# daisy9542/yolo-puncture

Measured on AMD Instinct MI355X. Metric: images/sec, higher is better.
Workload: dtype bf16

## Files before the change

yolo-puncture_amd/csrc/common.h:

```cpp
#pragma once
#include <hip/hip_runtime.h>
#include <stdint.h>
#include <string>
#include <vector>

namespace yp {

enum DType { DT_BF16 = 0, DT_F32 = 1 };
enum Act { ACT_NONE = 0, ACT_SILU = 1, ACT_RELU = 2 };

enum OpKind {
    OP_STEM = 0,
    OP_CONV = 1,
    OP_DWCONV = 2,
    OP_POOL5 = 3,
    OP_UPSAMPLE = 4,
    OP_ATTN = 5,
    OP_HEAD = 6,
    OP_CONVT = 7,
    OP_AMAX = 9,
    OP_POOL3 = 8,
};

struct View {
// ... 40 lines not shown
    int nlev = 0;
    double flops = 0, bytes = 0;
    std::string kernel;
    int cfg = -1;
    int fuse_dw = -1;
    bool fused = false;
    bool skip = false;
    int fuse_pre = -1;
    bool fused2 = false;
    int stem_op = -1;
    bool fused3 = false;
    int fold_up = -1;
    bool folded = false;
    int c2f_m1 = -1, c2f_m2 = -1;
    bool fused4 = false;
    int scd_pre = -1;
    bool fused5 = false;
    int fuse_tail = -1, tail_amax = -1;
    bool fused6 = false;
    int amax_post = -1;
    bool fused8 = false;
    int pw_pre = -1;
    bool fused7 = false;
    bool pw_store = false;
    int lane = 0;
    bool nms = false;
    int hb_box[3][3] = {{-1, -1, -1}, {-1, -1, -1}, {-1, -1, -1}}, hb_cf[3][3] = {{-1, -1, -1}, {-1, -1, -1}, {-1, -1, -1}};
    bool sparse_box = false, sparse_cf = false;
};

// ... 50 lines not shown
bool frontend_valid(const FrontParams& p);
hipError_t launch_frontend(const FrontParams& p, hipStream_t st);

struct C2fParams {
    const void* x; int x_stride, x_coff; size_t x_bytes;
    int B, H, W, C;
    const void* w1; const float* bias1; int act1, Kpad1; size_t w1_bytes;
    const void* w2; const float* bias2; int act2, Kpad2; size_t w2_bytes;
    int shortcut;
    const void* w3; const float* bias3; int act3, Kpad3, Cout; size_t w3_bytes;
    void* y; int y_stride, y_coff; size_t y_bytes;
    unsigned long long* clk;
};
bool c2f_fused_valid(const C2fParams& p);

struct ScdParams {
    const void* x; int x_stride, x_coff; size_t x_bytes; int B, H, W, K;
    const void* w1; const float* bias1; int act1, Kpad1, C; size_t w1_bytes;
    const void* wd; const float* biasd; int actd;
    void* y; int y_stride, y_coff; size_t y_bytes; int Ho, Wo;
    unsigned long long* clk;
};
bool scdown_fused_valid(const ScdParams& p);
const char* scdown_fused_kernel_name(const ScdParams& p);
bool scdown_stream_valid(const ScdParams& p);
const char* scdown_stream_kernel_name(const ScdParams& p);
hipError_t launch_scdown_stream(const ScdParams& p, hipStream_t st);
hipError_t launch_scdown_fused(const ScdParams& p, hipStream_t st);
hipError_t launch_c2f_fused(const C2fParams& p, hipStream_t st);

struct PoolParams {
    const void* x; int x_stride, x_coff;
    void* y; int y_stride, y_coff;
    int B, H, W, C;
};

struct UpParams {
    const void* x; int x_stride, x_coff;
    void* y; int y_stride, y_coff;
    int B, H, W, C;
};

struct AttnParams {
    const void* qkv; int q_stride, q_coff;
// ... 225 lines not shown
```

yolo-puncture_amd/csrc/engine.hip:

```cpp
#include "../../include/yolop.h"
#include "common.h"
#include <algorithm>
#include <array>
#include <chrono>

#include <cmath>
#include <cstdarg>
#include <cstdio>
#include <cstring>
#include <cstdlib>
#include <dlfcn.h>
#include <fcntl.h>
#include <fstream>
#include <map>
#include <sstream>
#include <memory>

using namespace yp;

static thread_local char g_err[512] = "";
static int fail(int code, const char* fmt, ...) {
    va_list ap;
    va_start(ap, fmt);
    vsnprintf(g_err, sizeof(g_err), fmt, ap);
// ... 17 lines not shown
    std::map<std::string, int> wmap;
    bool finalized = false;
    int pB = 0, pH = 0, pW = 0;
    bool planned = false, allocated = false;
    void* arena = nullptr;
    size_t arena_bytes = 0;
    int proto_t = -1;
    void* mask_ws = nullptr;
    void* head_ws = nullptr;
    size_t head_ws_bytes = 0;
    size_t mask_ws_bytes = 0;
    bool use_graph = false;
    bool graph_auto = false;
    std::map<std::array<int, 3>, bool> auto_replay;
    bool fuse = true;
    bool tail = false;
    bool sparse_head = true;
    void* sp_ws = nullptr; size_t sp_ws_bytes = 0;
    bool tune = true;
    int tune_source = 0;
    hipStream_t own_stream = nullptr;
    hipEvent_t ev_in = nullptr;
    hipGraphExec_t gexec = nullptr;
    hipGraph_t gsrc = nullptr;
    bool use_lanes = true;
    int n_captures = 0;
    int g_nodes = 0, g_edges = 0, g_edges_expected = 0;
    hipStream_t last_stream = nullptr; bool have_last = false;
    struct LaneStep { int op = -1; std::vector<int> waits; bool fork = false; bool record = false; };
    std::vector<LaneStep> lane_steps;
// ... 81 lines not shown
    int sdiv_of(View v) const { return e.tensors[v.t].sdiv; }

    void c2f(const std::string& p, View in, View out, int c2, int n, bool shortcut, bool cib, bool lk) {
        const int c = c2 / 2, sd = sdiv_of(in);
        const int Y = tensor(p + ".cat", (2 + n) * c, sd);
        int m1 = -1;
        conv(p + ".cv1", in, View{Y, 0, 2 * c}, 1, 1, ACT_SILU);
        for (int j = 0; j < n; ++j) {
            const View x{Y, (1 + j) * c, c}, y{Y, (2 + j) * c, c};
            const std::string q = p + ".m." + std::to_string(j);
            const View res = shortcut ? x : View{};
            if (!cib) {
                const int t = tensor(q + ".cv1", c, sd);
                conv(q + ".cv1", x, full(t), 3, 1, ACT_SILU);
                conv(q + ".cv2", full(t), y, 3, 1, ACT_SILU, res);
                if (n == 1) m1 = (int)e.ops.size() - 2;
            } else {
                const int t0 = tensor(q + ".cv1.0", c, sd), t1 = tensor(q + ".cv1.1", 2 * c, sd);
                const int t2 = tensor(q + ".cv1.2", 2 * c, sd), t3 = tensor(q + ".cv1.3", c, sd);
                dwconv(q + ".cv1.0", x, full(t0), 3, 1, ACT_SILU);
                conv(q + ".cv1.1", full(t0), full(t1), 1, 1, ACT_SILU);
                dwconv(q + ".cv1.2", full(t1), full(t2), lk ? 7 : 3, 1, ACT_SILU);
                conv(q + ".cv1.3", full(t2), full(t3), 1, 1, ACT_SILU);
                dwconv(q + ".cv1.4", full(t3), y, 3, 1, ACT_SILU, res);
            }
        }
        conv(p + ".cv2", full(Y), out, 1, 1, ACT_SILU);
        if (m1 >= 0) { e.ops.back().c2f_m1 = m1; e.ops.back().c2f_m2 = m1 + 1; }
    }
    void bottleneck(const std::string& q, View x, View y, int ch, bool shortcut) {
        const int t = tensor(q + ".cv1", ch, sdiv_of(x));
        conv(q + ".cv1", x, full(t), 3, 1, ACT_SILU);
        conv(q + ".cv2", full(t), y, 3, 1, ACT_SILU, shortcut ? x : View{});
    }
    void c3k2(const std::string& p, View in, View out, int c2, int n, bool c3k, double e) {
        const int c = (int)(c2 * e), sd = sdiv_of(in);
        const int Y = tensor(p + ".cat", (2 + n) * c, sd);
        conv(p + ".cv1", in, View{Y, 0, 2 * c}, 1, 1, ACT_SILU);
        for (int j = 0; j < n; ++j) {
            const View x{Y, (1 + j) * c, c}, y{Y, (2 + j) * c, c};
            const std::string q = p + ".m." + std::to_string(j);
            const int c_ = c / 2;
            if (!c3k) { bottleneck(q, x, y, c_, true); continue; }
            const int Z = tensor(q + ".cat", 2 * c_, sd);
            const int a0 = tensor(q + ".cv1", c_, sd), a1 = tensor(q + ".m.0", c_, sd);
            conv(q + ".cv1", x, full(a0), 1, 1, ACT_SILU);
            bottleneck(q + ".m.0", full(a0), full(a1), c_, true);
            bottleneck(q + ".m.1", full(a1), View{Z, 0, c_}, c_, true);
// ... 439 lines not shown
        if (d.in.coff < pw.out.coff || d.in.coff + d.in.C > pw.out.coff + pw.out.C) continue;
        if (e.tensors[pw.out.t].f32 || e.tensors[d.out.t].f32) continue;
        d.pw_pre = c;
    }
    return YP_OK;
}

static ConvParams conv_params(const yp_engine& e, const Op& o);
static void drop_graph(yp_engine& e) {
    if (e.gexec) { (void)hipGraphExecDestroy(e.gexec); e.gexec = nullptr; }
    if (e.gsrc) { (void)hipGraphDestroy(e.gsrc); e.gsrc = nullptr; }
}
static DwPwParams dwpw_params(const yp_engine& e, const Op& c);
static FrontParams front_params(const yp_engine& e, const Op& o, const uint8_t* img);
static C2fParams c2f_params(const yp_engine& e, const Op& o);
static ScdParams scd_params(const yp_engine& e, const Op& o);
static PwSpParams pwsp_params(const yp_engine& e, const Op& o);
static ClsOutParams cls_out_params(const yp_engine& e, const Op& o);
static bool views_overlap(const View& a, const View& b);
static size_t tensor_elem_bytes(const yp_engine& e, const TensorDesc& t) { return (t.f32 || e.dtype == DT_F32) ? 4 : 2; }

struct SparseWs {
    size_t sel, wlist, wcount, thr, box, cf, pcount, plist, t0box, t0cf, total;
    int plist_off[3], plist_cap[3];
    size_t t0_off[3];
    size_t rows;
};
static SparseWs sparse_ws_layout(int B, int max_det, const int (&HWl)[3]) {
    SparseWs w{};
    size_t off = 0;
// ... 75 lines not shown
            o.bytes += (double)w.cout * w.cin_g * w.k * w.k * es;
            if (o.kind == OP_STEM) o.bytes += (double)B * H * W * 3;
        } else if (o.kind == OP_ATTN) {
            const TensorDesc& ti = e.tensors[o.in.t];
            const double Nn = (double)ti.H * ti.W;
            o.flops = 2.0 * B * o.nh * Nn * Nn * (o.kd + o.hd);
        } else if (o.kind == OP_HEAD) {
            o.bytes = 0;
            for (int l = 0; l < 3; ++l) o.bytes += (o.amax[l].t >= 0) ? vbytes(o.amax[l]) : vbytes(o.cls[l]);
            o.bytes += (double)B * e.desc.max_det * (e.desc.nc + 64 + 6 + 1) * 4;
        }
    }
    e.pB = B; e.pH = H; e.pW = W; e.planned = true; e.allocated = false; e.warmed = false;
    for (auto& o : e.ops) o.cfg = -1;
    static const char* kn[] = {"stem_kernel", "", "dwconv_kernel", "pool5_kernel", "upsample2_kernel", "attention_kernel", "head_select_kernel", "", "sppf_pool3_kernel", "anchor_max_level_kernel"};
    for (auto& o : e.ops) { o.fused = false; o.skip = false; o.folded = false; o.fused2 = false; o.fused3 = false; o.fused4 = false; o.fused5 = false; o.fused6 = false; o.fused7 = false; o.fused8 = false; o.pw_store = false; o.sparse_box = false; o.sparse_cf = false; }
    static const bool no_fold = [] { const char* v = std::getenv("YOLOP_NO_FOLD"); return v && *v == '1'; }();
    for (auto& o : e.ops) {
        if (o.kind != OP_CONV || o.fold_up < 0 || e.dtype != DT_BF16 || no_fold) continue;
        o.folded = true;
        const ConvParams q = conv_params(e, o);
        bool any = false;
        for (int c = 0; c < conv_dma_p_num_cfgs() && !any; ++c) any = conv_dma_p_cfg_valid(q, c);
        if (any) e.ops[o.fold_up].skip = true;
        else o.folded = false;
    }
    for (auto& o : e.ops) {
        if (o.kind == OP_CONV && o.fuse_pre >= 0 && e.dtype == DT_BF16 && e.fuse) {
            o.fused2 = true;
            const int c = conv_halo_s2_pw_cfg(conv_params(e, o));
            if (c >= 0) {
// ... 54 lines not shown
            q.x_bytes = (size_t)B * q.H * q.W * q.x_stride * 2;
            if (dwconv_mfma_valid(q, e.dtype)) snprintf(buf, sizeof(buf), "dwconv_mfma_kernel<%d,%s>", o.k, B * (q.C / 32) >= 256 ? "false" : "true");
            else if (o.k == 3 && o.s == 1) snprintf(buf, sizeof(buf), "dwconv_row_kernel<%s,3,1,4>", t);
            else if (o.k == 3 && o.s == 2) snprintf(buf, sizeof(buf), "dwconv_row_kernel<%s,3,2,2>", t);
            else if (o.k == 7 && o.s == 1) snprintf(buf, sizeof(buf), "dwconv_row_kernel<%s,7,1,2>", t);
            else snprintf(buf, sizeof(buf), "dwconv_kernel<%s>", t);
            o.kernel = buf;
        } else if (o.kind == OP_STEM) {
            char buf[64];
            if (e.dtype == DT_BF16) snprintf(buf, sizeof(buf), "stem_mfma_kernel<%d>", o.out.C / 16);
            else snprintf(buf, sizeof(buf), "stem_kernel<f32>");
            o.kernel = buf;
        } else if (o.kind == OP_POOL3 && e.dtype == DT_BF16 && (o.in.C & 31) == 0) o.kernel = "sppf_pool3_bf16_kernel";
        else o.kernel = (o.kind == OP_HEAD && o.nms) ? "head_nms_kernel" : kn[o.kind];
    }
    for (auto& o : e.ops) {
        if (o.kind != OP_HEAD || o.nms || e.dtype != DT_BF16 || !e.sparse_head || e.desc.max_det > HEAD_MAXK || o.amax[0].t < 0) continue;
        for (int which = 0; which < 2; ++which) {
            const HeadBranchParams q = head_branch_params(e, o, which);
            if (q.cmid == 0 || !head_branch_valid(q)) continue;
            if (which == 1 && !o.sparse_box) continue;
            bool outside = false;
            for (int l = 0; l < 3 && !outside; ++l)
                for (int j = 0; j < 3 && !outside; ++j) {
                    const int oi = (which == 0 ? o.hb_box : o.hb_cf)[l][j];
                    const View& w = e.ops[oi].out;
                    for (size_t r = 0; r < e.ops.size() && !outside; ++r) {
                        const Op& q2 = e.ops[r];
                        if (&q2 == &o) continue;
                        bool member = false;
// ... 5 lines not shown
            if (outside) continue;
            (which == 0 ? o.sparse_box : o.sparse_cf) = true;
            for (int l = 0; l < 3; ++l)
                for (int j = 0; j < 3; ++j) {
                    Op& c = e.ops[(which == 0 ? o.hb_box : o.hb_cf)[l][j]];
                    c.skip = true;
                }
        }
    }
    {
        static const bool no_pwsp = [] { const char* v = std::getenv("YOLOP_NO_PWSP"); return v && *v == '1'; }();
        for (size_t i = 0; i < e.ops.size(); ++i) {
            Op& d = e.ops[i];
            if (d.pw_pre < 0 || e.dtype != DT_BF16 || !e.fuse || no_pwsp || d.skip || d.fused5) continue;
            Op& c = e.ops[d.pw_pre];
            if (c.skip || c.fused || c.fused2 || c.fused3 || c.fused4 || c.fused6 || c.folded) continue;
            bool between = false, other = false;
            for (size_t j = 0; j < e.ops.size(); ++j) {
                const Op& q = e.ops[j];
                if (j == i || (int)j == d.pw_pre || q.skip) continue;
                bool reads = false;
                for (const View* v : {&q.in, &q.res}) reads |= views_overlap(*v, c.out);
                if (q.kind == OP_HEAD)
                    for (int l = 0; l < 3; ++l) {
                        for (const View* v : {&q.box[l], &q.cls[l], &q.cf[l], &q.amax[l]}) reads |= views_overlap(*v, c.out);
                        for (int which = 0; which < 2; ++which) {
                            const int b0 = (which == 0 ? q.hb_box : q.hb_cf)[l][0];
                            if (b0 >= 0 && (which == 0 ? q.sparse_box : q.sparse_cf)) reads |= views_overlap(e.ops[b0].in, c.out);
                        }
                    }
                other |= reads;
// ... 1 lines not shown
                    between |= reads || views_overlap(q.out, c.out) || views_overlap(q.out, d.out) || views_overlap(q.out, d.res) || views_overlap(q.in, d.out) ||
                               views_overlap(q.res, d.out);
                }
            }
            if (between) continue;
            d.fused7 = true; d.pw_store = other;
            if (!pwsp_valid(pwsp_params(e, d))) { d.fused7 = false; d.pw_store = false; continue; }
            c.skip = true;
            d.kernel = pwsp_kernel_name(pwsp_params(e, d));
        }
    }
    {
        static const bool no_co = [] { const char* v = std::getenv("YOLOP_NO_CLSOUT"); return v && *v == '1'; }();
        for (auto& o : e.ops) {
            if (o.kind != OP_CONV || o.amax_post < 0 || e.dtype != DT_BF16 || !e.fuse || no_co) continue;
            if (o.skip || o.fused || o.fused2 || o.fused3 || o.fused4 || o.fused6 || o.folded || e.ops[o.amax_post].skip) continue;
            if (!cls_out_valid(cls_out_params(e, o))) continue;
            o.fused8 = true; e.ops[o.amax_post].skip = true;
            o.kernel = cls_out_kernel_name(cls_out_params(e, o));
        }
    }
    {
        const double es = e.es();
        auto vb = [&](const View& v) {
            if (v.t < 0) return 0.0;
            const TensorDesc& t = e.tensors[v.t];
            return (double)B * t.H * t.W * v.C * (double)tensor_elem_bytes(e, t);
        };
        auto wb = [&](const Op& q) { const WeightDesc& w = e.weights[q.widx]; return (double)w.cout * w.cin_g * w.k * w.k * es; };
        for (auto& o : e.ops) {
            if (o.kind == OP_DWCONV && o.fused5) { const Op& c1 = e.ops[o.scd_pre]; o.flops += c1.flops; o.bytes = vb(c1.in) + vb(o.out) + wb(c1) + wb(o); }
// ... 7 lines not shown
            else if (o.fused6) {
                const Op& c1 = e.ops[o.fuse_tail];
                const Op& d = e.ops[c1.fuse_dw];
                o.flops += c1.flops;
                o.bytes = vb(d.in) + vb(o.out) + wb(d) + wb(c1) + wb(o) + (o.tail_amax >= 0 ? vb(e.ops[o.tail_amax].out) : 0.0);
            }
            else if (o.fused3) {
                const Op &c1 = e.ops[o.fuse_pre], &st = e.ops[o.stem_op];
                o.flops += c1.flops + st.flops; o.bytes = (double)B * H * W * 3 + vb(o.out) + wb(st) + wb(c1) + wb(o);
            } else if (o.fused2) { const Op& c1 = e.ops[o.fuse_pre]; o.flops += c1.flops; o.bytes = vb(c1.in) + vb(o.out) + wb(c1) + wb(o); }
            else if (o.fused4) {
                const Op &m1 = e.ops[o.c2f_m1], &m2 = e.ops[o.c2f_m2];
                o.flops += m1.flops + m2.flops;
                o.bytes = vb(View{o.in.t, o.in.coff, 2 * m1.in.C}) + vb(o.out) + wb(m1) + wb(m2) + wb(o);
            }
            if (o.folded) { const Op& u = e.ops[o.fold_up]; o.bytes += vb(u.in) - vb(u.out); }
            if (o.fused8) o.bytes += vb(e.ops[o.amax_post].out);
        }
        for (auto& o : e.ops) {
            if (o.kind != OP_HEAD) continue;
            for (int which = 0; which < 2; ++which) {
                if (!(which == 0 ? o.sparse_box : o.sparse_cf)) continue;
                const HeadBranchParams q = head_branch_params(e, o, which);
                for (int l = 0; l < 3; ++l) {
                    const double nw = (double)B * e.desc.max_det / 3.0;
                    const double npos = std::min(9.0 * nw, (double)B * q.H[l] * q.W[l]);
                    o.flops += 2.0 * (npos * 9.0 * q.Cin[l] * q.cmid + nw * (9.0 * q.cmid * q.cmid + (double)q.cmid * q.cout));
                    o.bytes += npos * (9.0 * q.Cin[l] * 2 + 2.0 * q.cmid * 2) + nw * q.cout * 4 + (9.0 * q.Cin[l] * q.cmid + 9.0 * q.cmid * q.cmid + q.cmid * q.cout) * 2;
                }
            }
// ... 115 lines not shown

static FrontParams front_params(const yp_engine& e, const Op& o, const uint8_t* img) {
    const Op& c1 = e.ops[o.fuse_pre];
    const Op& st = e.ops[o.stem_op];
    const WeightDesc &w0 = e.weights[st.widx], &w1 = e.weights[c1.widx], &w2 = e.weights[o.widx];
    const TensorDesc &t0 = e.tensors[st.out.t], &to = e.tensors[o.out.t];
    FrontParams p{};
    p.img = img; p.imgH = e.pH; p.imgW = e.pW; p.B = e.pB;
    p.w0 = w0.d_w2; p.bias0 = w0.d_b; p.act0 = st.act; p.C0 = st.out.C; p.H1 = t0.H; p.W1 = t0.W;
    p.w1 = w1.d_w; p.bias1 = w1.d_b; p.act1 = c1.act; p.C1 = c1.out.C; p.Kpad1 = w1.Kpad; p.w1_bytes = w1.mat_bytes;
    p.w2 = w2.d_w; p.bias2 = w2.d_b; p.act2 = o.act; p.C2 = o.out.C; p.Kpad2 = w2.Kpad; p.w2_bytes = w2.mat_bytes;
    p.y = to.ptr; p.y_stride = to.C; p.y_coff = o.out.coff; p.y_bytes = to.bytes; p.Ho = to.H; p.Wo = to.W;
    return p;
}

static C2fParams c2f_params(const yp_engine& e, const Op& o) {
    const Op &m1 = e.ops[o.c2f_m1], &m2 = e.ops[o.c2f_m2];
    const WeightDesc &w1 = e.weights[m1.widx], &w2 = e.weights[m2.widx], &w3 = e.weights[o.widx];
    const TensorDesc &ti = e.tensors[o.in.t], &to = e.tensors[o.out.t];
    C2fParams p{};
    p.x = ti.ptr; p.x_stride = ti.C; p.x_coff = o.in.coff; p.x_bytes = ti.bytes; p.B = e.pB; p.H = ti.H; p.W = ti.W; p.C = m1.in.C;
    p.w1 = w1.d_w; p.bias1 = w1.d_b; p.act1 = m1.act; p.Kpad1 = w1.Kpad; p.w1_bytes = w1.mat_bytes;
    p.w2 = w2.d_w; p.bias2 = w2.d_b; p.act2 = m2.act; p.Kpad2 = w2.Kpad; p.w2_bytes = w2.mat_bytes;
    p.shortcut = m2.res.t >= 0 ? 1 : 0;
    p.w3 = w3.d_w; p.bias3 = w3.d_b; p.act3 = o.act; p.Kpad3 = w3.Kpad; p.Cout = o.out.C; p.w3_bytes = w3.mat_bytes;
    p.y = to.ptr; p.y_stride = to.C; p.y_coff = o.out.coff; p.y_bytes = to.bytes;
    if (m1.in.t != o.in.t || m1.in.coff != o.in.coff + p.C || m2.out.t != o.in.t || m2.out.coff != o.in.coff + 2 * p.C || o.in.C != 3 * p.C ||
        m1.k != 3 || m2.k != 3 || m1.s != 1 || m2.s != 1 || m1.out.C != p.C || m2.out.C != p.C || m1.res.t >= 0 ||
        (m2.res.t >= 0 && (m2.res.t != m1.in.t || m2.res.coff != m1.in.coff)) || (to.f32 && e.dtype == DT_BF16)) p.C = 0;
    return p;
// ... 59 lines not shown
    auto T = [&](const View& v) -> const TensorDesc& { return e.tensors[v.t]; };
    const int B = e.pB;
    switch (o.kind) {
        case OP_STEM: {
            const WeightDesc& w = e.weights[o.widx];
            const TensorDesc& to = T(o.out);
            StemParams p{};
            p.x = a.in; p.H = e.pH; p.W = e.pW; p.w = (const float*)w.d_w; p.wpk = w.d_w2; p.bias = w.d_b;
            p.y = to.ptr; p.y_stride = to.C; p.y_coff = o.out.coff; p.Ho = to.H; p.Wo = to.W; p.C0 = o.out.C; p.B = B; p.act = o.act;
            return launch_stem(p, e.dtype, st);
        }
        case OP_CONV:
            if (o.fused || o.fused6) return launch_conv_dwpw(dwpw_params(e, o), st);
            if (o.fused3) return launch_frontend(front_params(e, o, a.in), st);
            if (o.fused4) return launch_c2f_fused(c2f_params(e, o), st);
            if (o.fused2) { const ConvParams q = conv_params(e, o); return launch_conv_halo_s2(q, o.cfg - 500, st); }
            if (o.fused8) return launch_cls_out(cls_out_params(e, o), st);
            if (o.cfg == PWSP_CFG) return launch_pwsp(pwsp_params(e, o), st);
            if (conv_dma_forced_cfg() == PWSP_CFG && e.dtype == DT_BF16 && !o.folded) {
                const PwSpParams q = pwsp_params(e, o);
                if (q.sp == 0 && pwsp_valid(q)) return launch_pwsp(q, st);
            }
            return launch_conv(conv_params(e, o), e.dtype, st);
        case OP_CONVT: {
            const WeightDesc& w = e.weights[o.widx];
            const TensorDesc &ti = T(o.in), &to = T(o.out);
            for (int dy = 0; dy < 2; ++dy)
                for (int dx = 0; dx < 2; ++dx) {
                    ConvParams p{};
                    p.x = ti.ptr; p.x_stride = ti.C; p.x_coff = o.in.coff; p.H = ti.H; p.W = ti.W; p.Cin = o.in.C;
// ... 135 lines not shown
            }
            hipError_t ee;
            if ((ee = hipEventRecord(e0, nullptr)) != hipSuccess) return ee;
            hipError_t err = run_op(e, o, none, nullptr);
            if (err != hipSuccess) return err;
            if ((ee = hipEventRecord(e1, nullptr)) != hipSuccess) return ee;
            if ((ee = hipEventSynchronize(e1)) != hipSuccess) return ee;
            float ms = 0;
            if ((ee = hipEventElapsedTime(&ms, e0, e1)) != hipSuccess) return ee;
            if (rep > 0) tmin = std::min(tmin, ms);
        }
        return hipSuccess;
    };
    for (Op& o : e.ops) {
        if (o.kind != OP_CONV && o.kind != OP_CONVT) continue;
        if (o.fused || o.fused2 || o.fused4 || o.fused6 || o.fused8 || o.skip) continue;
        ConvParams p{};
        if (o.kind == OP_CONV) p = conv_params(e, o);
        else { p.Cin = o.in.C; p.Cout = o.out.C; p.ks = 1; p.Kpad = e.weights[o.widx].Kpad; p.M = e.pB * e.tensors[o.in.t].H * e.tensors[o.in.t].W;
               p.x_bytes = e.tensors[o.in.t].bytes; p.w_bytes = e.weights[o.widx].mat_bytes; }
        if (!conv_dma_supported(p)) continue;
        float best = 1e30f;
        int bestc = -1;
        std::vector<std::pair<float, int>> timed;
        for (int c = 0; c < conv_dma_num_cfgs(); ++c) {
            if (p.x2_C > 0 || !conv_dma_cfg_valid(p, c)) continue;
            o.cfg = c;
            float tmin;
            hipError_t err = time_cfg(o, tmin);
            if (err != hipSuccess) return fail(YP_ERR_HIP, "autotune op %s cfg %d: %s", o.name.c_str(), c, hipGetErrorString(err));
            timed.emplace_back(tmin, c);
// ... 81 lines not shown
    os << pre << "_f" << e.desc.family << (char)e.desc.variant << (e.desc.task ? "seg" : "det") << "_nc" << e.desc.nc << "_dt" << e.dtype << "_" << e.pB << "x" << e.pH << "x" << e.pW
       << "_t" << TUNE_TABLE_VERSION << ".txt";
    return os.str();
}
static ConvParams tune_params(const yp_engine& e, const Op& o) {
    if (o.kind == OP_CONV) return conv_params(e, o);
    ConvParams p{};
    p.Cin = o.in.C; p.Cout = o.out.C; p.ks = 1; p.Kpad = e.weights[o.widx].Kpad; p.M = e.pB * e.tensors[o.in.t].H * e.tensors[o.in.t].W;
    p.x_bytes = e.tensors[o.in.t].bytes; p.w_bytes = e.weights[o.widx].mat_bytes;
    return p;
}
static bool apply_tuning(yp_engine& e, const int* cfgs, int n) {
    if (n != (int)e.ops.size()) return false;
    for (size_t i = 0; i < e.ops.size(); ++i) {
        const Op& o = e.ops[i];
        if ((o.kind != OP_CONV && o.kind != OP_CONVT) || o.fused || o.fused2 || o.fused4 || o.fused6 || o.fused8 || o.skip) continue;
        ConvParams p = tune_params(e, o);
        p.cfg = -1;
        if (cfgs[i] == PWSP_CFG) { if (o.kind != OP_CONV || o.folded || !pwsp_valid(pwsp_params(e, o))) return false; continue; }
        if (!conv_cfg_usable(p, e.dtype, cfgs[i])) return false;
    }
    for (size_t i = 0; i < e.ops.size(); ++i) {
        Op& o = e.ops[i];
        if ((o.kind != OP_CONV && o.kind != OP_CONVT) || o.fused || o.fused2 || o.fused4 || o.fused6 || o.fused8 || o.skip) continue;
        o.cfg = cfgs[i];
        if (o.cfg == PWSP_CFG) { o.kernel = pwsp_kernel_name(pwsp_params(e, o)); continue; }
        ConvParams p = tune_params(e, o);
        p.cfg = o.cfg;
        o.kernel = conv_kernel_name(p, e.dtype);
    }
    return true;
}
static bool load_tune_cache(yp_engine& e, bool packaged = false) {
    const std::string path = tune_cache_path(e, packaged);
    if (path.empty()) return false;
    std::ifstream f(path);
    if (!f) return false;
    std::map<std::string, int> m;
    std::string name;
// ... 58 lines not shown
        o.kernel += ">";
    }
}

static bool views_overlap(const View& a, const View& b) {
    return a.t >= 0 && a.t == b.t && a.coff < b.coff + b.C && b.coff < a.coff + a.C;
}
static void op_views(const yp_engine& e, const Op& o, std::vector<View>& rd, std::vector<View>& wr) {
    rd.clear(); wr.clear();
    if (o.skip) return;
    if (o.fused) rd.push_back(e.ops[o.fuse_dw].in);
    else if (o.fused6) rd.push_back(e.ops[e.ops[o.fuse_tail].fuse_dw].in);
    else if (o.fused5) rd.push_back(e.ops[o.scd_pre].in);
    else if (o.fused7) rd.push_back(e.ops[o.pw_pre].in);
    else if (o.fused4) rd.push_back(View{o.in.t, o.in.coff, 2 * e.ops[o.c2f_m1].in.C});
    else if (o.fused3) {  }
    else if (o.fused2) rd.push_back(e.ops[o.fuse_pre].in);
    else if (o.in.t >= 0) rd.push_back(o.in);
    if (o.folded) rd.push_back(e.ops[o.fold_up].in);
    if (o.res.t >= 0) rd.push_back(o.res);
    if (o.out.t >= 0) wr.push_back(o.out);
    if (o.fused7 && o.pw_store) wr.push_back(e.ops[o.pw_pre].out);
    if (o.fused8) wr.push_back(e.ops[o.amax_post].out);
    if (o.fused6 && o.tail_amax >= 0) wr.push_back(e.ops[o.tail_amax].out);
    if (o.kind == OP_HEAD)
        for (int l = 0; l < 3; ++l) {
            if (o.sparse_box) rd.push_back(e.ops[o.hb_box[l][0]].in);
            else if (o.box[l].t >= 0) rd.push_back(o.box[l]);
            if (o.cls[l].t >= 0) rd.push_back(o.cls[l]);
            if (o.sparse_cf) rd.push_back(e.ops[o.hb_cf[l][0]].in);
// ... 248 lines not shown
        if (sigaction(g_fatal_sigs[i], &sa, &g_prev_sa[i]) != 0) g_prev_sa[i].sa_handler = SIG_DFL;
    }
}

int yp_create(const yp_model_desc* desc, int device, yp_engine** out) {
    if (!desc || !out) return fail(YP_ERR_ARG, "null argument");
    if (desc->nc <= 0 || desc->max_det <= 0 || desc->max_det > 1024) return fail(YP_ERR_ARG, "bad nc/max_det");
    if (desc->task == YP_TASK_SEGMENT && desc->max_det > YP_MAX_MASKS)
        return fail(YP_ERR_ARG, "segmentation engines take max_det <= %d (the mask tail keeps one frame's coefficients in LDS; ultralytics' default is 300)", YP_MAX_MASKS);
    if (desc->dtype != YP_BF16 && desc->dtype != YP_F32) return fail(YP_ERR_ARG, "bad dtype");
    if (desc->task != YP_TASK_DETECT && desc->task != YP_TASK_SEGMENT) return fail(YP_ERR_ARG, "bad task");
    install_fatal_handlers();
    std::unique_ptr<yp_engine> e(new yp_engine());
    e->desc = *desc; e->device = device; e->dtype = desc->dtype;
    { const char* nf = std::getenv("YOLOP_NO_FUSE"); e->fuse = !(nf && *nf == '1'); }
    { const char* tf = std::getenv("YOLOP_TAIL"); e->tail = tf && *tf == '1'; }
    { const char* dh = std::getenv("YOLOP_DENSE_HEAD"); e->sparse_head = !(dh && *dh == '1'); }
    int rc = build_graph(*e);
    if (rc != YP_OK) return rc;
    for (const Op& o : e->ops)
        for (const View* v : {&o.in, &o.out, &o.res})
            if (v->t >= 0 && o.kind != OP_STEM && ((v->C & 7) || (v->coff & 7)) && !e->tensors[v->t].f32)
                return fail(YP_ERR_ARG, "op %s: channel slice (%d,%d) is not a multiple of 8", o.name.c_str(), v->coff, v->C);
    *out = e.release();
    return YP_OK;
}

int yp_destroy(yp_engine* e) {
    if (!e) return YP_OK;
    if (e->finalized || e->arena) { (void)hipSetDevice(e->device); (void)hipDeviceSynchronize(); }
// ... 472 lines not shown
    if (!e->planned) return fail(YP_ERR_STATE, "yp_plan has not been called");
    size_t acc = 0;
    if (!e->finalized)
        for (WeightDesc& w : e->weights) {
            if (!w.have_w || !w.have_b || w.w.empty()) continue;
            std::vector<unsigned char> main, aux;
            pack_weight(*e, w, main, aux);
            acc += main.size() + aux.size();
        }
    for (const Op& o : e->ops) {
        if (o.skip) continue;
        if (o.kind == OP_CONV) {
            if (o.fused || o.fused6) acc += (size_t)dwpw_params(*e, o).Cout;
            else if (o.fused3) acc += (size_t)front_params(*e, o, nullptr).C2;
            else if (o.fused4) acc += (size_t)c2f_params(*e, o).Cout;
            else acc += (size_t)conv_params(*e, o).Cout;
        } else if (o.kind == OP_DWCONV && o.fused5) acc += (size_t)scd_params(*e, o).C;
        else if (o.fused7) acc += (size_t)pwsp_params(*e, o).C1;
    }
    finish_kernel_names(*e);
    save_tune_cache(*e);
    (void)load_tune_cache(*e);
    {
        const std::string tp = tune_cache_path(*e, true);
        if (!tp.empty() && std::ifstream(tp).good()) {
            std::vector<std::pair<int, std::string>> keep;
            for (const Op& o : e->ops) keep.emplace_back(o.cfg, o.kernel);
            const bool ok = load_tune_cache(*e, true);
            for (size_t i = 0; i < e->ops.size(); ++i) { e->ops[i].cfg = keep[i].first; e->ops[i].kernel = keep[i].second; }
            if (!ok) return fail(YP_ERR_STATE, "packaged tune table %s does not apply to this build's plan", tp.c_str());
// ... 207 lines not shown
```

Measured before the change: 22530.

## Fuse bottleneck 3x3 conv pairs into a single LDS-resident kernel

Adds a fused kernel for bottleneck blocks with 128 channels. It computes the first 3x3 conv over a halo tile and keeps its output in LDS, then runs the second 3x3 conv, the residual add and the store in the same launch. Weights stream through a three-stage LDS pipeline using buffer-to-LDS loads and MFMA. This removes the intermediate tensor round trip through global memory and one kernel launch per bottleneck, at the cost of recomputing halo pixels. Tile geometry is picked by a simple cost model.

```diff
diff --git a/yolo-puncture_amd/csrc/bneck_fused.hip b/yolo-puncture_amd/csrc/bneck_fused.hip
--- /dev/null
+++ b/yolo-puncture_amd/csrc/bneck_fused.hip
@@ -0,0 +1,335 @@
+#include "common.h"
+#include <cstdio>
+#include <cstdlib>
+#include <type_traits>
+
+namespace yp {
+
+typedef __attribute__((ext_vector_type(8))) __bf16 bf16x8;
+typedef __attribute__((ext_vector_type(4))) float f32x4;
+typedef __attribute__((address_space(3))) void lds_void;
+
+template <int N> __device__ __forceinline__ void bn_wait_vm() {
+    static_assert(N >= 0 && N < 64, "vmcnt range");
+    __builtin_amdgcn_s_waitcnt((N & 0xF) | (7 << 4) | (0xF << 8) | (((N >> 4) & 3) << 14));
+}
+__device__ __forceinline__ int bswz(int row) { return ((row >> 2) & 1) << 1; }
+
+constexpr int BN_C = 128;
+constexpr int BN_NS = 3;
+constexpr int BN_FM1 = 5;
+constexpr int BN_FM2 = 4;
+constexpr int BN_SW = 3 * BN_C * 64;
+constexpr int BN_MAXPPC = (160 * 1024 - BN_NS * BN_SW) / (4 * 1024);
+constexpr int BN_NCLK = 6;
+
+struct BneckGeo { int TR, TC, tiles_h, tiles_w, ppc, tpc; };
+
+__device__ unsigned long long g_bn_clk[8][BN_NCLK];
+__device__ int g_bn_abl;
+
+template <bool RES, bool CLK>
+__global__ __launch_bounds__(512) void c2f_fused_kernel(const BneckParams p, const BneckGeo g) {
+#define BN_STAMP(i) do { if (CLK && blockIdx.x == 0 && (threadIdx.x & 63) == 0) g_bn_clk[threadIdx.x >> 6][i] = wall_clock64(); } while (0)
+    BN_STAMP(0);
+    const int abl = CLK ? g_bn_abl : 0;
+    constexpr int FN = 4, NW = 8;
+    constexpr unsigned OOB = 0x80000000u;
+    extern __shared__ __attribute__((aligned(1024))) unsigned char smem[];
+    unsigned char* const Xs = smem;
+    unsigned char* const Ws = smem + (size_t)4 * g.ppc * 1024;
+
+    const int tid = threadIdx.x, lane = tid & 63;
+    const int wave = __builtin_amdgcn_readfirstlane(tid >> 6);
+    const int wm = wave >> 1, wn = wave & 1;
+    const int fr = lane & 15, fc = lane >> 4;
+
+    int t = blockIdx.x;
+    const int tw = t % g.tiles_w; t /= g.tiles_w;
+    const int th = t % g.tiles_h;
+    const int b = t / g.tiles_h;
+    const int r0 = th * g.TR, c0 = tw * g.TC;
+    const int HC = g.TC + 4, RC = g.TC + 2;
+    const int nring = (g.TR + 2) * RC, npix = g.TR * g.TC;
+
+    const __amdgpu_buffer_rsrc_t xrs = __builtin_amdgcn_make_buffer_rsrc((void*)p.x, 0, (int)p.x_bytes, 0x00020000);
+    const __amdgpu_buffer_rsrc_t w1rs = __builtin_amdgcn_make_buffer_rsrc((void*)p.w1, 0, (int)p.w1_bytes, 0x00020000);
+    const __amdgpu_buffer_rsrc_t w2rs = __builtin_amdgcn_make_buffer_rsrc((void*)p.w2, 0, (int)p.w2_bytes, 0x00020000);
+    const __amdgpu_buffer_rsrc_t yrs = __builtin_amdgcn_make_buffer_rsrc((void*)p.y, 0, (int)p.y_bytes, 0x00020000);
+
+    f32x4 acc1[FN][BN_FM1];
+#pragma unroll
+    for (int a = 0; a < FN; ++a) {
+        const int co = wn * (FN * 16) + a * 16 + fc * 4;
+        const f32x4 bv = f32x4{p.bias1[co], p.bias1[co + 1], p.bias1[co + 2], p.bias1[co + 3]};
+#pragma unroll
+        for (int f = 0; f < BN_FM1; ++f) acc1[a][f] = bv;
+    }
+    auto issue_x = [&](int ch) {
+        const int npx = (g.TR + 4) * HC;
+        for (int pi = wave; pi < g.ppc; pi += NW) {
+            const int hp = pi * 16 + (lane >> 2), pc = lane & 3;
+            const int c8 = pc ^ bswz(hp);
+            const int hy = hp / HC, hx = hp - hy * HC;
+            const int hi = r0 - 2 + hy, wi = c0 - 2 + hx;
+            const bool ok = hp < npx && (unsigned)hi < (unsigned)p.H && (unsigned)wi < (unsigned)p.W;
+            const unsigned voff = ok ? (unsigned)((((b * p.H + hi) * p.W + wi) * p.x_stride + p.x_coff + ch * 32 + c8 * 8) * 2) : OOB;
+            __builtin_amdgcn_raw_ptr_buffer_load_lds(xrs, (lds_void*)(Xs + (ch * g.ppc + pi) * 1024), 16, voff, 0, 0, 0);
+        }
+    };
+    constexpr int NST = 24;
+    unsigned wbase[3];
+#pragma unroll
+    for (int j = 0; j < 3; ++j) {
+        const int q = wave + j * NW;
+        const int kx = q >> 3, n = (q & 7) * 16 + (lane >> 2), pc = lane & 3;
+        const int c8 = pc ^ bswz(n);
+        wbase[j] = (unsigned)((n * p.Kpad1 + kx * BN_C + c8 * 8) * 2);
+    }
+    auto issue_piece = [&](int j, int s) {
+        const int cv = s >= 12, sl = s - cv * 12, ch = sl / 3, ky = sl - ch * 3;
+        if (CLK && (abl & 1) && s >= 2) return;
+        const unsigned voff = (s < NST) ? wbase[j] + (unsigned)((ky * 3 * BN_C + ch * 32) * 2) : OOB;
+        __builtin_amdgcn_raw_ptr_buffer_load_lds(cv ? w2rs : w1rs, (lds_void*)(Ws + (s % BN_NS) * BN_SW + (wave + j * NW) * 1024), 16, voff, 0, 0, 0);
+    };
+    issue_x(0);
+#pragma unroll
+    for (int j = 0; j < 3; ++j) issue_piece(j, 0);
+#pragma unroll
+    for (int j = 0; j < 3; ++j) issue_piece(j, 1);
+
+    auto frag_range = [&](int nfr, int& f0, int& myf) {
+        const int base = nfr >> 2, ext = nfr & 3;
+        f0 = wm * base + min(wm, ext);
+        myf = base + (wm < ext ? 1 : 0);
+    };
+    const int nfr1 = (nring + 15) >> 4, nfr2 = (npix + 15) >> 4;
+    int f01, myf1, f02, myf2;
+    frag_range(nfr1, f01, myf1);
+    frag_range(nfr2, f02, myf2);
+    myf1 = __builtin_amdgcn_readfirstlane(myf1); myf2 = __builtin_amdgcn_readfirstlane(myf2);
+    unsigned lb1[BN_FM1], lb2[BN_FM2];
+#pragma unroll
+    for (int f = 0; f < BN_FM1; ++f) {
+        const int rp = min((f01 + f) * 16 + fr, nring - 1);
+        const int r = rp / RC, c = rp - r * RC;
+        lb1[f] = (unsigned)((r * HC + c) * 64 + fc * 16);
+    }
+#pragma unroll
+    for (int f = 0; f < BN_FM2; ++f) {
+        const int pp = min((f02 + f) * 16 + fr, npix - 1);
+        const int r = pp / g.TC, c = pp - r * g.TC;
+        lb2[f] = (unsigned)((r * RC + c) * 64 + fc * 16);
+    }
+    unsigned wl[3][FN];
+#pragma unroll
+    for (int kx = 0; kx < 3; ++kx)
+#pragma unroll
+        for (int a = 0; a < FN; ++a) {
+            const int rw = kx * BN_C + wn * (FN * 16) + a * 16 + fr;
+            wl[kx][a] = (unsigned)(rw * 64 + ((fc ^ bswz(rw)) * 16));
+        }
+
+    const unsigned xs_l = (unsigned)(size_t)(__attribute__((address_space(3))) unsigned char*)Xs;
+    const unsigned ws_l = (unsigned)(size_t)(__attribute__((address_space(3))) unsigned char*)Ws;
+    auto lds_rd = [](bf16x8& dst, unsigned addr) { asm volatile("ds_read_b128 %0, %1" : "=v"(dst) : "v"(addr)); };
+    auto hold = [](bf16x8& r) { asm volatile("" : "+v"(r)); };
+
+    auto run_conv = [&](int s0, auto FMc, f32x4 (&acc)[FN][decltype(FMc)::value], const unsigned (&lb)[decltype(FMc)::value], int myf, unsigned plane_bytes, int pitch) {
+        constexpr int FM = decltype(FMc)::value;
+        constexpr int RD = FN + FM;
+        bf16x8 xf[2][FM], wf[2][FN];
+        auto read_tap = [&](bf16x8 (&xd)[FM], bf16x8 (&wd)[FN], int s, int kx) {
+            if (CLK && (abl & 4)) return;
+            const int sl = s % 12, ch = sl / 3, ky = sl - ch * 3;
+            const unsigned wsb = ws_l + (unsigned)((s % BN_NS) * BN_SW);
+#pragma unroll
+            for (int a = 0; a < FN; ++a) lds_rd(wd[a], wsb + wl[kx][a]);
+            const unsigned xsb = xs_l + (unsigned)ch * plane_bytes;
+            const unsigned tapb = (unsigned)((ky * pitch + kx) * 64);
+#pragma unroll
+            for (int f = 0; f < FM; ++f) {
+                const unsigned L = lb[f] + tapb;
+                lds_rd(xd[f], xsb + (L ^ ((L >> 3) & 32u)));
+            }
+        };
+        auto wait_set = [&](auto Nc, bf16x8 (&xd)[FM], bf16x8 (&wd)[FN]) {
+            constexpr int N = decltype(Nc)::value;
+            asm volatile("s_waitcnt lgkmcnt(%0)" : : "n"(N) : "memory");
+#pragma unroll
+            for (int f = 0; f < FM; ++f) hold(xd[f]);
+#pragma unroll
+            for (int a = 0; a < FN; ++a) hold(wd[a]);
+        };
+        auto mfma_tap = [&](bf16x8 (&xd)[FM], bf16x8 (&wd)[FN]) {
+            if (CLK && (abl & 2)) return;
+#pragma unroll
+            for (int f = 0; f < FM; ++f) {
+                if (f >= myf) break;
+#pragma unroll
+                for (int a = 0; a < FN; ++a) acc[a][f] = __builtin_amdgcn_mfma_f32_16x16x32_bf16(wd[a], xd[f], acc[a][f], 0, 0, 0);
+            }
+        };
+        auto barrier_for = [&](int s) {
+            bn_wait_vm<3>();
+            __builtin_amdgcn_s_barrier();
+            const int sl = s % 12, ch = sl / 3, ky = sl - ch * 3;
+            if (s < 12 && ky == 0 && ch + 1 < 4) issue_x(ch + 1);
+        };
+        auto stage = [&](int s, auto Pc) {
+            constexpr int A = decltype(Pc)::value, B = A ^ 1;
+            read_tap(xf[B], wf[B], s, 1);
+            wait_set(std::integral_constant<int, RD>{}, xf[A], wf[A]);
+            mfma_tap(xf[A], wf[A]);
+            issue_piece(0, s + 2);
+            read_tap(xf[A], wf[A], s, 2);
+            wait_set(std::integral_constant<int, RD>{}, xf[B], wf[B]);
+            mfma_tap(xf[B], wf[B]);
+            issue_piece(1, s + 2);
+            issue_piece(2, s + 2);
+            wait_set(std::integral_constant<int, 0>{}, xf[A], wf[A]);
+            if (s + 1 < s0 + 12) {
+                barrier_for(s + 1);
+                read_tap(xf[B], wf[B], s + 1, 0);
+            }
+            mfma_tap(xf[A], wf[A]);
+        };
+        barrier_for(s0);
+        if (s0 == 0) BN_STAMP(1);
+        read_tap(xf[0], wf[0], s0, 0);
+        for (int s = s0; s < s0 + 12; s += 2) {
+            stage(s, std::integral_constant<int, 0>{});
+            stage(s + 1, std::integral_constant<int, 1>{});
+        }
+    };
+
+    run_conv(0, std::integral_constant<int, BN_FM1>{}, acc1, lb1, myf1, (unsigned)g.ppc * 1024u, HC);
+    BN_STAMP(2);
+    __builtin_amdgcn_s_barrier();
+#pragma unroll
+    for (int f = 0; f < BN_FM1; ++f) {
+        if (f >= myf1) break;
+        const int rp = (f01 + f) * 16 + fr;
+        const int r = rp / RC, c = rp - r * RC;
+        const int hi = r0 - 1 + r, wi = c0 - 1 + c;
+        const bool inside = (unsigned)hi < (unsigned)p.H && (unsigned)wi < (unsigned)p.W;
+        if (rp >= nring) continue;
+#pragma unroll
+        for (int a = 0; a < FN; ++a) {
+            const int co = wn * (FN * 16) + a * 16 + fc * 4;
+            float v[4] = {acc1[a][f][0], acc1[a][f][1], acc1[a][f][2], acc1[a][f][3]};
+            if (p.act1 == ACT_SILU) silu4_packed(v);
+            __attribute__((aligned(8))) __bf16 o[4] = {(__bf16)v[0], (__bf16)v[1], (__bf16)v[2], (__bf16)v[3]};
+            unsigned long long bits = *(const unsigned long long*)o;
+            if (!inside) bits = 0ull;
+            const int cw = co & 31, c8 = cw >> 3;
+            const unsigned addr = xs_l + (unsigned)((co >> 5) * g.tpc * 1024 + rp * 64 + ((c8 ^ bswz(rp)) << 4) + (cw & 7) * 2);
+            asm volatile("ds_write_b64 %0, %1" ::"v"(addr), "v"(bits) : "memory");
+        }
+    }
+    asm volatile("s_waitcnt lgkmcnt(0)" ::: "memory");
+    BN_STAMP(3);
+
+    f32x4 acc2[FN][BN_FM2];
+#pragma unroll
+    for (int a = 0; a < FN; ++a) {
+        const int co = wn * (FN * 16) + a * 16 + fc * 4;
+        const f32x4 bv = f32x4{p.bias2[co], p.bias2[co + 1], p.bias2[co + 2], p.bias2[co + 3]};
+#pragma unroll
+        for (int f = 0; f < BN_FM2; ++f) acc2[a][f] = bv;
+    }
+    run_conv(12, std::integral_constant<int, BN_FM2>{}, acc2, lb2, myf2, (unsigned)g.tpc * 1024u, RC);
+    BN_STAMP(4);
+#pragma unroll
+    for (int f = 0; f < BN_FM2; ++f) {
+        if (f >= myf2) break;
+        const int pp = (f02 + f) * 16 + fr;
+        const int r = pp / g.TC, c = pp - r * g.TC;
+        const int ho = r0 + r, wo = c0 + c;
+        const bool pix_ok = pp < npix && ho < p.H && wo < p.W;
+        const unsigned m = (unsigned)((b * p.H + ho) * p.W + wo);
+#pragma unroll
+        for (int a = 0; a < FN; ++a) {
+            const int co = wn * (FN * 16) + a * 16 + fc * 4;
+            float v[4] = {acc2[a][f][0], acc2[a][f][1], acc2[a][f][2], acc2[a][f][3]};
+            if (p.act2 == ACT_SILU) silu4_packed(v);
+            if (RES) {
+                const uint2 rr = pix_ok ? *(const uint2*)((const __bf16*)p.res + (size_t)m * p.res_stride + p.res_coff + co) : make_uint2(0u, 0u);
+                v[0] += __uint_as_float(rr.x << 16); v[1] += __uint_as_float(rr.x & 0xffff0000u);
+                v[2] += __uint_as_float(rr.y << 16); v[3] += __uint_as_float(rr.y & 0xffff0000u);
+            }
+            const unsigned off = pix_ok ? (m * (unsigned)p.y_stride + (unsigned)(p.y_coff + co)) * 2u : OOB;
+            __attribute__((aligned(8))) __bf16 o[4] = {(__bf16)v[0], (__bf16)v[1], (__bf16)v[2], (__bf16)v[3]};
+            __builtin_amdgcn_raw_buffer_store_b64(*(const __attribute__((ext_vector_type(2))) unsigned*)o, yrs, off, 0, 0);
+        }
+    }
+    BN_STAMP(5);
+    bn_wait_vm<0>();
+#undef BN_STAMP
+}
+
+static bool bneck_geometry(const BneckParams& p, BneckGeo& g) {
+    bool found = false;
+    double best = 1e30;
+    for (int TR = 1; TR <= p.H; ++TR)
+        for (int TC = 4; TC <= p.W; ++TC) {
+            const int ppc = ((TR + 4) * (TC + 4) + 15) / 16;
+            if (ppc > BN_MAXPPC) break;
+            const int nfr1 = ((TR + 2) * (TC + 2) + 15) / 16, nfr2 = (TR * TC + 15) / 16;
+            if (nfr1 > 4 * BN_FM1 || nfr2 > 4 * BN_FM2) break;
+            const int th = (p.H + TR - 1) / TR, tw = (p.W + TC - 1) / TC;
+            const long tiles = (long)p.B * th * tw;
+            const long rounds = (tiles + 255) / 256;
+            const double cost = rounds * ((nfr1 + 1) / 2 + (nfr2 + 1) / 2 + 6.0) + tiles * 1e-6;
+            if (cost < best) { best = cost; g = BneckGeo{TR, TC, th, tw, ppc, ((TR + 2) * (TC + 2) + 15) / 16}; found = true; }
+        }
+    return found;
+}
+
+bool bneck_fused_valid(const BneckParams& p) {
+    if (p.C != BN_C || p.Kpad1 != 9 * BN_C || p.Kpad2 != 9 * BN_C || p.B <= 0 || p.H <= 0 || p.W <= 0) return false;
+    if ((p.x_stride & 7) || (p.x_coff & 7) || (p.y_stride & 3) || (p.y_coff & 3) || (p.res && ((p.res_stride & 3) || (p.res_coff & 3)))) return false;
+    if (p.x_bytes >= (1ull << 31) || p.y_bytes >= (1ull << 31) || p.w1_bytes >= (1ull << 31) || p.w2_bytes >= (1ull << 31)) return false;
+    if (p.w1_bytes < (size_t)BN_C * p.Kpad1 * 2 || p.w2_bytes < (size_t)BN_C * p.Kpad2 * 2) return false;
+    if ((p.act1 != ACT_NONE && p.act1 != ACT_SILU) || (p.act2 != ACT_NONE && p.act2 != ACT_SILU)) return false;
+    BneckGeo g;
+    return bneck_geometry(p, g);
+}
+
+const char* bneck_fused_kernel_name(const BneckParams& p) { return p.res ? "c2f_fused_kernel<true,false>" : "c2f_fused_kernel<false,false>"; }
+
+template <bool RES, bool CLK>
+static hipError_t launch_bneck_var(const BneckParams& p, const BneckGeo& g, hipStream_t st) {
+    auto kern = c2f_fused_kernel<RES, CLK>;
+    static bool attr = false;
+    if (!attr) {
+        hipError_t e = hipFuncSetAttribute((const void*)kern, hipFuncAttributeMaxDynamicSharedMemorySize, (int)(160 * 1024));
+        if (e != hipSuccess) return e;
+        attr = true;
+    }
+    const size_t sh = (size_t)4 * g.ppc * 1024 + (size_t)BN_NS * BN_SW;
+    hipLaunchKernelGGL(kern, dim3(p.B * g.tiles_h * g.tiles_w), dim3(512), sh, st, p, g);
+    return hipGetLastError();
+}
+
+hipError_t launch_bneck_fused(const BneckParams& p, hipStream_t st) {
+    BneckGeo g;
+    if (!bneck_geometry(p, g)) return hipErrorInvalidValue;
+    static const bool clocks = [] { const char* v = std::getenv("YOLOP_BNECK_CLOCKS"); return v && *v == '1'; }();
+    if (clocks) {
+        { const char* v = std::getenv("YOLOP_BNECK_ABL"); const int ab = v ? atoi(v) : 0; (void)hipMemcpyToSymbol(HIP_SYMBOL(g_bn_abl), &ab, sizeof(int)); }
+        hipError_t e = p.res ? launch_bneck_var<true, true>(p, g, st) : launch_bneck_var<false, true>(p, g, st);
+        if (e != hipSuccess) return e;
+        if ((e = hipStreamSynchronize(st)) != hipSuccess) return e;
+        unsigned long long h[8][BN_NCLK];
+        (void)hipMemcpyFromSymbol(h, HIP_SYMBOL(g_bn_clk), sizeof(h));
+        double ph[BN_NCLK - 1] = {};
+        for (int w = 0; w < 8; ++w) for (int i = 0; i + 1 < BN_NCLK; ++i) ph[i] += (double)(h[w][i + 1] - h[w][i]) / 100.0 / 8.0;
+        fprintf(stderr, "[bneck clocks] %dx%d res %d tile %dx%d: fill %.2f us, cv1 %.2f us, t epilogue %.2f us, cv2 %.2f us, stores %.2f us (workgroup 0, mean of 8 waves)\n",
+                p.H, p.W, p.res ? 1 : 0, g.TR, g.TC, ph[0], ph[1], ph[2], ph[3], ph[4]);
+        return hipSuccess;
+    }
+    return p.res ? launch_bneck_var<true, false>(p, g, st) : launch_bneck_var<false, false>(p, g, st);
+}
+
+}
diff --git a/yolo-puncture_amd/csrc/common.h b/yolo-puncture_amd/csrc/common.h
--- a/yolo-puncture_amd/csrc/common.h
+++ b/yolo-puncture_amd/csrc/common.h
@@ -78,6 +78,8 @@
     bool folded = false;
     int c2f_m1 = -1, c2f_m2 = -1;
     bool fused4 = false;
+    int bneck_pre = -1;
+    bool fused9 = false;
     int scd_pre = -1;
     bool fused5 = false;
     int fuse_tail = -1, tail_amax = -1;
@@ -158,6 +160,17 @@
 };
 bool c2f_fused_valid(const C2fParams& p);
 
+struct BneckParams {
+    const void* x; int x_stride, x_coff; size_t x_bytes;
+    int B, H, W, C;
+    const void* w1; const float* bias1; int act1, Kpad1; size_t w1_bytes;
+    const void* w2; const float* bias2; int act2, Kpad2; size_t w2_bytes;
+    const void* res; int res_stride, res_coff;
+    void* y; int y_stride, y_coff; size_t y_bytes;
+};
+bool bneck_fused_valid(const BneckParams& p);
+const char* bneck_fused_kernel_name(const BneckParams& p);
+
 struct ScdParams {
     const void* x; int x_stride, x_coff; size_t x_bytes; int B, H, W, K;
     const void* w1; const float* bias1; int act1, Kpad1, C; size_t w1_bytes;
@@ -172,6 +185,7 @@
 hipError_t launch_scdown_stream(const ScdParams& p, hipStream_t st);
 hipError_t launch_scdown_fused(const ScdParams& p, hipStream_t st);
 hipError_t launch_c2f_fused(const C2fParams& p, hipStream_t st);
+hipError_t launch_bneck_fused(const BneckParams& p, hipStream_t st);
 
 struct PoolParams {
     const void* x; int x_stride, x_coff;
diff --git a/yolo-puncture_amd/csrc/engine.hip b/yolo-puncture_amd/csrc/engine.hip
--- a/yolo-puncture_amd/csrc/engine.hip
+++ b/yolo-puncture_amd/csrc/engine.hip
@@ -55,6 +55,7 @@
     bool graph_auto = false;
     std::map<std::array<int, 3>, bool> auto_replay;
     bool fuse = true;
+    bool bneck = true;
     bool tail = false;
     bool sparse_head = true;
     void* sp_ws = nullptr; size_t sp_ws_bytes = 0;
@@ -166,6 +167,7 @@
                 const int t = tensor(q + ".cv1", c, sd);
                 conv(q + ".cv1", x, full(t), 3, 1, ACT_SILU);
                 conv(q + ".cv2", full(t), y, 3, 1, ACT_SILU, res);
+                e.ops.back().bneck_pre = (int)e.ops.size() - 2;
                 if (n == 1) m1 = (int)e.ops.size() - 2;
             } else {
                 const int t0 = tensor(q + ".cv1.0", c, sd), t1 = tensor(q + ".cv1.1", 2 * c, sd);
@@ -184,6 +186,7 @@
         const int t = tensor(q + ".cv1", ch, sdiv_of(x));
         conv(q + ".cv1", x, full(t), 3, 1, ACT_SILU);
         conv(q + ".cv2", full(t), y, 3, 1, ACT_SILU, shortcut ? x : View{});
+        e.ops.back().bneck_pre = (int)e.ops.size() - 2;
     }
     void c3k2(const std::string& p, View in, View out, int c2, int n, bool c3k, double e) {
         const int c = (int)(c2 * e), sd = sdiv_of(in);
@@ -653,6 +656,7 @@
 static DwPwParams dwpw_params(const yp_engine& e, const Op& c);
 static FrontParams front_params(const yp_engine& e, const Op& o, const uint8_t* img);
 static C2fParams c2f_params(const yp_engine& e, const Op& o);
+static BneckParams bneck_params(const yp_engine& e, const Op& o);
 static ScdParams scd_params(const yp_engine& e, const Op& o);
 static PwSpParams pwsp_params(const yp_engine& e, const Op& o);
 static ClsOutParams cls_out_params(const yp_engine& e, const Op& o);
@@ -758,7 +762,7 @@
     e.pB = B; e.pH = H; e.pW = W; e.planned = true; e.allocated = false; e.warmed = false;
     for (auto& o : e.ops) o.cfg = -1;
     static const char* kn[] = {"stem_kernel", "", "dwconv_kernel", "pool5_kernel", "upsample2_kernel", "attention_kernel", "head_select_kernel", "", "sppf_pool3_kernel", "anchor_max_level_kernel"};
-    for (auto& o : e.ops) { o.fused = false; o.skip = false; o.folded = false; o.fused2 = false; o.fused3 = false; o.fused4 = false; o.fused5 = false; o.fused6 = false; o.fused7 = false; o.fused8 = false; o.pw_store = false; o.sparse_box = false; o.sparse_cf = false; }
+    for (auto& o : e.ops) { o.fused = false; o.skip = false; o.folded = false; o.fused2 = false; o.fused3 = false; o.fused4 = false; o.fused5 = false; o.fused6 = false; o.fused7 = false; o.fused8 = false; o.fused9 = false; o.pw_store = false; o.sparse_box = false; o.sparse_cf = false; }
     static const bool no_fold = [] { const char* v = std::getenv("YOLOP_NO_FOLD"); return v && *v == '1'; }();
     for (auto& o : e.ops) {
         if (o.kind != OP_CONV || o.fold_up < 0 || e.dtype != DT_BF16 || no_fold) continue;
@@ -843,6 +847,27 @@
         } else if (o.kind == OP_POOL3 && e.dtype == DT_BF16 && (o.in.C & 31) == 0) o.kernel = "sppf_pool3_bf16_kernel";
         else o.kernel = (o.kind == OP_HEAD && o.nms) ? "head_nms_kernel" : kn[o.kind];
     }
+    {
+        for (size_t i = 0; i < e.ops.size(); ++i) {
+            Op& o = e.ops[i];
+            if (o.kind != OP_CONV || o.bneck_pre < 0 || e.dtype != DT_BF16 || !e.fuse || !e.bneck || conv_dma_forced_cfg() >= 0) continue;
+            Op& c1 = e.ops[o.bneck_pre];
+            if (o.skip || c1.skip || o.fused || o.fused2 || o.fused4 || o.fused6 || o.fused8 || o.folded || c1.fused || c1.fused2 || c1.folded) continue;
+            bool other = false;
+            for (size_t j = 0; j < e.ops.size() && !other; ++j) {
+                if (j == i || (int)j == o.bneck_pre) continue;
+                const Op& q = e.ops[j];
+                for (const View* v : {&q.in, &q.res}) other |= views_overlap(*v, c1.out);
+                if (q.kind == OP_HEAD)
+                    for (int l = 0; l < 3; ++l)
+                        for (const View* v : {&q.box[l], &q.cls[l], &q.cf[l], &q.amax[l]}) other |= views_overlap(*v, c1.out);
+            }
+            if (other) continue;
+            const BneckParams q = bneck_params(e, o);
+            if (!bneck_fused_valid(q)) continue;
+            o.fused9 = true; c1.skip = true; o.kernel = bneck_fused_kernel_name(q);
+        }
+    }
     for (auto& o : e.ops) {
         if (o.kind != OP_HEAD || o.nms || e.dtype != DT_BF16 || !e.sparse_head || e.desc.max_det > HEAD_MAXK || o.amax[0].t < 0) continue;
         for (int which = 0; which < 2; ++which) {
@@ -878,7 +903,7 @@
             Op& d = e.ops[i];
             if (d.pw_pre < 0 || e.dtype != DT_BF16 || !e.fuse || no_pwsp || d.skip || d.fused5) continue;
             Op& c = e.ops[d.pw_pre];
-            if (c.skip || c.fused || c.fused2 || c.fused3 || c.fused4 || c.fused6 || c.folded) continue;
+            if (c.skip || c.fused || c.fused2 || c.fused3 || c.fused4 || c.fused6 || c.fused9 || c.folded) continue;
             bool between = false, other = false;
             for (size_t j = 0; j < e.ops.size(); ++j) {
                 const Op& q = e.ops[j];
@@ -910,7 +935,7 @@
         static const bool no_co = [] { const char* v = std::getenv("YOLOP_NO_CLSOUT"); return v && *v == '1'; }();
         for (auto& o : e.ops) {
             if (o.kind != OP_CONV || o.amax_post < 0 || e.dtype != DT_BF16 || !e.fuse || no_co) continue;
-            if (o.skip || o.fused || o.fused2 || o.fused3 || o.fused4 || o.fused6 || o.folded || e.ops[o.amax_post].skip) continue;
+            if (o.skip || o.fused || o.fused2 || o.fused3 || o.fused4 || o.fused6 || o.fused9 || o.folded || e.ops[o.amax_post].skip) continue;
             if (!cls_out_valid(cls_out_params(e, o))) continue;
             o.fused8 = true; e.ops[o.amax_post].skip = true;
             o.kernel = cls_out_kernel_name(cls_out_params(e, o));
@@ -948,6 +973,7 @@
                 o.flops += m1.flops + m2.flops;
                 o.bytes = vb(View{o.in.t, o.in.coff, 2 * m1.in.C}) + vb(o.out) + wb(m1) + wb(m2) + wb(o);
             }
+            else if (o.fused9) { const Op& c1 = e.ops[o.bneck_pre]; o.flops += c1.flops; o.bytes = vb(c1.in) + vb(o.res) + vb(o.out) + wb(c1) + wb(o); }
             if (o.folded) { const Op& u = e.ops[o.fold_up]; o.bytes += vb(u.in) - vb(u.out); }
             if (o.fused8) o.bytes += vb(e.ops[o.amax_post].out);
         }
@@ -1093,6 +1119,21 @@
     return p;
 }
 
+static BneckParams bneck_params(const yp_engine& e, const Op& o) {
+    const Op& c1 = e.ops[o.bneck_pre];
+    const WeightDesc &w1 = e.weights[c1.widx], &w2 = e.weights[o.widx];
+    const TensorDesc &ti = e.tensors[c1.in.t], &tt = e.tensors[c1.out.t], &to = e.tensors[o.out.t];
+    BneckParams p{};
+    p.x = ti.ptr; p.x_stride = ti.C; p.x_coff = c1.in.coff; p.x_bytes = ti.bytes; p.B = e.pB; p.H = ti.H; p.W = ti.W; p.C = c1.in.C;
+    p.w1 = w1.d_w; p.bias1 = w1.d_b; p.act1 = c1.act; p.Kpad1 = w1.Kpad; p.w1_bytes = w1.mat_bytes;
+    p.w2 = w2.d_w; p.bias2 = w2.d_b; p.act2 = o.act; p.Kpad2 = w2.Kpad; p.w2_bytes = w2.mat_bytes;
+    if (o.res.t >= 0) { p.res = e.tensors[o.res.t].ptr ? e.tensors[o.res.t].ptr : (const void*)1; p.res_stride = e.tensors[o.res.t].C; p.res_coff = o.res.coff; }
+    p.y = to.ptr; p.y_stride = to.C; p.y_coff = o.out.coff; p.y_bytes = to.bytes;
+    if (c1.k != 3 || o.k != 3 || c1.s != 1 || o.s != 1 || c1.out.C != p.C || o.in.C != p.C || o.out.C != p.C || !(o.in.t == c1.out.t && o.in.coff == c1.out.coff) ||
+        c1.res.t >= 0 || w1.cin_pad > c1.in.C || w2.cin_pad > o.in.C || tt.H != ti.H || tt.W != ti.W || to.H != ti.H || to.W != ti.W || to.f32) p.C = 0;
+    return p;
+}
+
 static C2fParams c2f_params(const yp_engine& e, const Op& o) {
     const Op &m1 = e.ops[o.c2f_m1], &m2 = e.ops[o.c2f_m2];
     const WeightDesc &w1 = e.weights[m1.widx], &w2 = e.weights[m2.widx], &w3 = e.weights[o.widx];
@@ -1182,6 +1223,7 @@
             if (o.fused || o.fused6) return launch_conv_dwpw(dwpw_params(e, o), st);
             if (o.fused3) return launch_frontend(front_params(e, o, a.in), st);
             if (o.fused4) return launch_c2f_fused(c2f_params(e, o), st);
+            if (o.fused9) return launch_bneck_fused(bneck_params(e, o), st);
             if (o.fused2) { const ConvParams q = conv_params(e, o); return launch_conv_halo_s2(q, o.cfg - 500, st); }
             if (o.fused8) return launch_cls_out(cls_out_params(e, o), st);
             if (o.cfg == PWSP_CFG) return launch_pwsp(pwsp_params(e, o), st);
@@ -1347,7 +1389,7 @@
     };
     for (Op& o : e.ops) {
         if (o.kind != OP_CONV && o.kind != OP_CONVT) continue;
-        if (o.fused || o.fused2 || o.fused4 || o.fused6 || o.fused8 || o.skip) continue;
+        if (o.fused || o.fused2 || o.fused4 || o.fused6 || o.fused8 || o.fused9 || o.skip) continue;
         ConvParams p{};
         if (o.kind == OP_CONV) p = conv_params(e, o);
         else { p.Cin = o.in.C; p.Cout = o.out.C; p.ks = 1; p.Kpad = e.weights[o.widx].Kpad; p.M = e.pB * e.tensors[o.in.t].H * e.tensors[o.in.t].W;
@@ -1459,7 +1501,7 @@
     if (n != (int)e.ops.size()) return false;
     for (size_t i = 0; i < e.ops.size(); ++i) {
         const Op& o = e.ops[i];
-        if ((o.kind != OP_CONV && o.kind != OP_CONVT) || o.fused || o.fused2 || o.fused4 || o.fused6 || o.fused8 || o.skip) continue;
+        if ((o.kind != OP_CONV && o.kind != OP_CONVT) || o.fused || o.fused2 || o.fused4 || o.fused6 || o.fused8 || o.fused9 || o.skip) continue;
         ConvParams p = tune_params(e, o);
         p.cfg = -1;
         if (cfgs[i] == PWSP_CFG) { if (o.kind != OP_CONV || o.folded || !pwsp_valid(pwsp_params(e, o))) return false; continue; }
@@ -1467,7 +1509,7 @@
     }
     for (size_t i = 0; i < e.ops.size(); ++i) {
         Op& o = e.ops[i];
-        if ((o.kind != OP_CONV && o.kind != OP_CONVT) || o.fused || o.fused2 || o.fused4 || o.fused6 || o.fused8 || o.skip) continue;
+        if ((o.kind != OP_CONV && o.kind != OP_CONVT) || o.fused || o.fused2 || o.fused4 || o.fused6 || o.fused8 || o.fused9 || o.skip) continue;
         o.cfg = cfgs[i];
         if (o.cfg == PWSP_CFG) { o.kernel = pwsp_kernel_name(pwsp_params(e, o)); continue; }
         ConvParams p = tune_params(e, o);
@@ -1556,6 +1598,7 @@
     else if (o.fused5) rd.push_back(e.ops[o.scd_pre].in);
     else if (o.fused7) rd.push_back(e.ops[o.pw_pre].in);
     else if (o.fused4) rd.push_back(View{o.in.t, o.in.coff, 2 * e.ops[o.c2f_m1].in.C});
+    else if (o.fused9) rd.push_back(e.ops[o.bneck_pre].in);
     else if (o.fused3) {  }
     else if (o.fused2) rd.push_back(e.ops[o.fuse_pre].in);
     else if (o.in.t >= 0) rd.push_back(o.in);
@@ -1834,6 +1877,7 @@
     std::unique_ptr<yp_engine> e(new yp_engine());
     e->desc = *desc; e->device = device; e->dtype = desc->dtype;
     { const char* nf = std::getenv("YOLOP_NO_FUSE"); e->fuse = !(nf && *nf == '1'); }
+    { const char* nb = std::getenv("YOLOP_NO_BNECK"); e->bneck = !(nb && *nb == '1'); }
     { const char* tf = std::getenv("YOLOP_TAIL"); e->tail = tf && *tf == '1'; }
     { const char* dh = std::getenv("YOLOP_DENSE_HEAD"); e->sparse_head = !(dh && *dh == '1'); }
     int rc = build_graph(*e);
@@ -2336,6 +2380,7 @@
             if (o.fused || o.fused6) acc += (size_t)dwpw_params(*e, o).Cout;
             else if (o.fused3) acc += (size_t)front_params(*e, o, nullptr).C2;
             else if (o.fused4) acc += (size_t)c2f_params(*e, o).Cout;
+            else if (o.fused9) acc += (size_t)bneck_params(*e, o).C;
             else acc += (size_t)conv_params(*e, o).Cout;
         } else if (o.kind == OP_DWCONV && o.fused5) acc += (size_t)scd_params(*e, o).C;
         else if (o.fused7) acc += (size_t)pwsp_params(*e, o).C1;
```

Result: no change. 22730 (median of 6 runs) (+0.9%).
